# PetarKirov/Chess2RT

Measured on AMD Instinct MI355X. Metric: Mray/s (reference-equivalent rays per second: one primary ray per sample + one shadow ray per (hit, lit light), counted as the reference casts them; ms/frame in ms_per_step), higher is better.
Workload: dtype f64; 1 GPU; lecture5.sdl 3840x2160, 5 tap(s)/pixel (AAEnabled as shipped: reference 5-tap AA), dof off; primary_rays_per_frame=41472000, full=False

## Files before the change

### chess2rt_amd/csrc/c2rt_device.h

```cpp
#ifndef C2RT_DEVICE_H
#define C2RT_DEVICE_H

#include <stddef.h>
#include <stdint.h>

#include "../../include/c2rt.h"
#include "csg_void.h"

namespace c2rt {

constexpr int kMaxCsgHits = C2RT_MAX_CSG_HITS;
constexpr int kCsgEntries = 2 * kMaxCsgHits;
constexpr int kTileW = 8, kTileH = 8;
constexpr int kWave = 64;
inline size_t padded_grid_blocks(uint32_t tile_rows, uint32_t blocks_x) { return (size_t)((tile_rows + 7u) / 8u * 8u) * blocks_x; }
constexpr int kMaxCullNodes = 32;
constexpr int kHullEdges = 6;
constexpr int kMaxCullLights = 4;
constexpr int kWavesPerBlock = 1;
constexpr int kBlockThreads = kWave * kWavesPerBlock;
constexpr int kCsgLdsPerEntry = kWave * (8 + 2);
constexpr int kCsgFullCap(int levels) { return kCsgEntries * (levels > 0 ? levels : 1); }
constexpr int kCsgFirstCap(int levels) { return levels <= 2 ? 16 : 20; }
static_assert(3 * kWavesPerBlock * kCsgFirstCap(C2RT_MAX_CSG_DEPTH) * kCsgLdsPerEntry <= 160 * 1024, "three workgroups per CU");

enum GeomFlags : int32_t {
    kGeomBounded = 1,
    kCsgShortA = 2,
    kCsgShortB = 4,
    kGeomFinite = 8,
    kCsgCertain = 16,
};

struct alignas(16) DevGeom {
    int32_t type, left, right;
    int32_t flags;
    double p[4];
    double bound[4];
    double q[6];
};

enum NodeFlags : uint32_t {
    kNodeIdentityMatrix = 1u,
    kNodeZeroOffset = 2u,
    kNodeAxisPlane = 4u,
    kNodePlaneNormal = 8u,
    kNodeCsgTile = 16u,
};

struct alignas(16) DevMat {
    int32_t shader_type;
    int32_t tex_type;
    int32_t tex;
    float strength;
    float color[3];
    uint32_t pad;
    double exponent;
    uint32_t pad2[2];
    uint32_t texdata[8];
};

struct alignas(16) DevNode {
    int32_t geom, shader;
    uint32_t flags, pad;
    double off[3];
    double pad2;
    DevGeom g;
    double inv[9];
    double m[9];
    double tinv[9];
    double pad3;
    DevMat mat;
};

struct alignas(16) DevShader {
    int32_t type, tex;
    float color[3];
    float strength;
    double exponent;
};

struct alignas(16) DevTex {
    int32_t type;
    uint32_t width, height;
    float scaling;
    uint64_t offset;
    float color[18];
    double param[6];
};

struct alignas(16) DevLight {
    double pos[3];
    float color[3];
    uint32_t lit;
    uint32_t equal;
    uint32_t pad;
};

struct RenderParams {
    const DevGeom *geoms;
    const DevNode *nodes;
    const DevShader *shaders;
    const DevTex *textures;
    const DevLight *lights;
// ... 89 lines not shown
```

### chess2rt_amd/csrc/c2rt_kernels.hip

```cpp
#include "c2rt_trace_common.inc"

namespace c2rt {
namespace {

constexpr int kLeanMaxLevels = 3;

template <int LEVELS, int DOF, bool MLC, int PO, bool CNT>
DEV void render_one(const RenderParams &P, KArgs K, const uint32_t b)
{
    if constexpr (CNT || LEVELS > kLeanMaxLevels) {
        exact::render_tile<LEVELS, DOF, MLC, PO, CNT>(P, K, b);
    } else {
        if (!P.force_exact) {
            const bool redo = lean::render_tile<LEVELS, DOF, MLC, PO, false>(P, K, b);
            if (!__ballot(redo)) return;
            if (threadIdx.x % kWave == 0) atomicAdd(P.redo_counter, 1ull);
        }
        if constexpr (LEVELS <= 1 && !DOF && PO != kSpecPlanes) {
            KArgs K2 = K;
            uint32_t b2 = b;
            asm volatile("" : "+s"(K2), "+s"(b2));
            exact::render_tile<LEVELS, DOF, MLC, PO, false>(*(const RenderParams *)K2, K2, b2);
        } else {
            exact::render_tile<LEVELS, DOF, MLC, PO, false>(P, K, b);
// ... 86 lines not shown

#if C2RT_UNIT == 5
__global__ void deinterleave_kernel(const float *__restrict__ gathered, float *__restrict__ frame,
                                    uint32_t row_floats, uint32_t strip_height, uint32_t world, uint32_t rows_pad)
{
    const uint32_t y = blockIdx.y;
    const uint32_t strip = y / strip_height;
    const uint32_t rank = strip % world;
    const uint32_t lr = (strip / world) * strip_height + y % strip_height;
    const float *src = gathered + ((size_t)rank * rows_pad + lr) * (size_t)row_floats;
    float *dst = frame + (size_t)y * row_floats;
    if ((row_floats & 3u) == 0) {
        const float4 *s4 = reinterpret_cast<const float4 *>(src);
        float4 *d4 = reinterpret_cast<float4 *>(dst);
        for (uint32_t i = blockIdx.x * blockDim.x + threadIdx.x; i < row_floats / 4; i += gridDim.x * blockDim.x) d4[i] = s4[i];
    } else {
        for (uint32_t i = blockIdx.x * blockDim.x + threadIdx.x; i < row_floats; i += gridDim.x * blockDim.x) dst[i] = src[i];
    }
}

__global__ void encode_rgb32_kernel(const float *__restrict__ frame, uint32_t *__restrict__ out, uint64_t n,
                                    const uint8_t *__restrict__ lut)
{
    for (uint64_t i = (uint64_t)blockIdx.x * blockDim.x + threadIdx.x; i < n; i += (uint64_t)gridDim.x * blockDim.x) {
        uint32_t ch[3];
#pragma unroll
        for (int c = 0; c < 3; ++c) {
            const float x = frame[3 * i + c];
            ch[c] = !(x > 0) ? 0u : (x >= 1 ? 255u : (uint32_t)lut[(int)(x * 4096.0f)]);
        }
        out[i] = ch[2] | (ch[1] << 8) | (ch[0] << 16);
    }
}

DEV void tile_masks_body(const RenderParams &P, KArgs K, const VoidCull &V, const SphereCull &S, const DarkCull *D, uint32_t *table, uint32_t tile_rows)
{
    const uint32_t i = blockIdx.x * blockDim.x + threadIdx.x;
    const uint32_t cols = P.blocks_x * kWavesPerBlock;
    const uint32_t trow = i / cols, tcol = i % cols;
    if (trow >= tile_rows) return;
    uint32_t m[8];
    tile_mask_entry(P, K, V, S, D, trow, tcol, m);
    typedef uint32_t __attribute__((ext_vector_type(4))) u4_t;
    u4_t v, w;
    v.x = m[0]; v.y = m[1]; v.z = m[2]; v.w = m[3];
    w.x = m[4]; w.y = m[5]; w.z = m[6]; w.w = m[7];
    const size_t slot = tile_mask_slot(P, trow, tcol);
    reinterpret_cast<u4_t *>(table)[slot] = v;
    if (P.n_cull_lights > 1u) reinterpret_cast<u4_t *>(table)[(size_t)P.mask_entries + slot] = w;
}

static_assert(sizeof(RenderParams) + sizeof(VoidCull) + sizeof(SphereCull) + 24 <= 4096, "the kernel-argument segment holds at most 4 KiB");
__global__ void __launch_bounds__(256) tile_masks_kernel(const RenderParams P, const VoidCull V, const SphereCull S, const DarkCull *dark,
                                                         uint32_t *__restrict__ table, uint32_t tile_rows)
{
    const DarkCull C2RT_K *D = (const DarkCull C2RT_K *)dark;
    tile_masks_body(P, (KArgs)__builtin_amdgcn_kernarg_segment_ptr(), V, S, (const DarkCull *)D, table, tile_rows);
}

__global__ void __launch_bounds__(256) tile_masks_batch_kernel(const RenderParams *table, const BatchCull *culls)
{
    const KArgs K = batch_block(table);
    const BatchCull C2RT_K *C = (const BatchCull C2RT_K *)culls + blockIdx.y;
    asm volatile("" : "+s"(C));
    const RenderParams &P = *(const RenderParams *)K;
    if (!P.n_cull || !P.tile_masks) return;
    const BatchCull &B = *(const BatchCull *)C;
    tile_masks_body(P, K, B.v, B.s, &B.d, const_cast<uint32_t *>(P.tile_masks), (P.mask_rows + kTileH - 1) / kTileH);
}
#endif

}

#ifndef C2RT_UNIT
#error "compile with -DC2RT_UNIT=0..5 (see Makefile)"
#endif

#if C2RT_UNIT >= 0 && C2RT_UNIT <= C2RT_MAX_CSG_DEPTH

static uint32_t frame_grid_x(const RenderParams &p)
{
    return p.retry_mode ? 2048u : (uint32_t)padded_grid_blocks(p.tiles_y, p.blocks_x);
}
static size_t frame_lds(const RenderParams &p) { return (size_t)p.csg_cap * kCsgLdsPerEntry * kWavesPerBlock; }

template <>
int launch_render_level<C2RT_UNIT>(const RenderParams &p, bool dof_or_stereo, void *stream)
{
    hipStream_t s = static_cast<hipStream_t>(stream);
    const dim3 grid(frame_grid_x(p)), block(kBlockThreads);
    const size_t lds = frame_lds(p);
    const bool stereo = p.cam.stereo_separation != 0;
    const bool multi = p.n_lights > 1;
    const bool idn = p.all_identity && !p.ray_counters;
#define C2RT_LAUNCH(KERNEL, ...)                                                                        \
    do {                                                                                                \
        if (p.ray_counters) hipLaunchKernelGGL((KERNEL<__VA_ARGS__, true>), grid, block, lds, s, p);    \
        else hipLaunchKernelGGL((KERNEL<__VA_ARGS__, false>), grid, block, lds, s, p);                  \
    } while (0)
#if C2RT_UNIT == 0
    if (p.planes_only && !multi) {
        if (dof_or_stereo && stereo) C2RT_LAUNCH(render_kernel_planes, 2);
        else if (dof_or_stereo) C2RT_LAUNCH(render_kernel_planes, 1);
        else C2RT_LAUNCH(render_kernel_planes, 0);
        return (int)hipGetLastError();
    }
#endif
    if (dof_or_stereo) {
        if (stereo) C2RT_LAUNCH(render_kernel_dof, C2RT_UNIT, true, 2);
        else if (multi) C2RT_LAUNCH(render_kernel_dof, C2RT_UNIT, true, 1);
        else C2RT_LAUNCH(render_kernel_dof, C2RT_UNIT, false, 1);
    } else if (multi) {
        C2RT_LAUNCH(render_kernel, C2RT_UNIT, 0, true);
    } else if (idn) {
        hipLaunchKernelGGL((render_kernel_idn<C2RT_UNIT>), grid, block, lds, s, p);
    } else {
        C2RT_LAUNCH(render_kernel, C2RT_UNIT, 0, false);
    }
#undef C2RT_LAUNCH
    return (int)hipGetLastError();
}

template <>
int launch_render_batch_level<C2RT_UNIT>(const RenderParams &p0, const RenderParams *table_dev, uint32_t n_frames, void *stream)
{
    hipStream_t s = static_cast<hipStream_t>(stream);
    const dim3 grid(frame_grid_x(p0), n_frames), block(kBlockThreads);
    const size_t lds = frame_lds(p0);
#if C2RT_UNIT == 0
    if (p0.planes_only && p0.n_lights <= 1) {
        hipLaunchKernelGGL(render_kernel_planes_batch, grid, block, lds, s, table_dev);
        return (int)hipGetLastError();
    }
#endif
    if (p0.n_lights > 1) hipLaunchKernelGGL((render_kernel_batch<C2RT_UNIT, true>), grid, block, lds, s, table_dev);
    else if (p0.all_identity) hipLaunchKernelGGL((render_kernel_idn_batch<C2RT_UNIT>), grid, block, lds, s, table_dev);
    else hipLaunchKernelGGL((render_kernel_batch<C2RT_UNIT, false>), grid, block, lds, s, table_dev);
    return (int)hipGetLastError();
}

#elif C2RT_UNIT == 5

int launch_render_batch(const RenderParams &p0, const KernelVariant &v, const RenderParams *table_dev, uint32_t n_frames, void *stream)
{
    if (v.dof_or_stereo || p0.ray_counters || !n_frames || n_frames > 65535u) return (int)hipErrorInvalidValue;
    return for_csg_levels(v.csg_levels, [&](auto L) { return launch_render_batch_level<decltype(L)::value>(p0, table_dev, n_frames, stream); });
}

int launch_tile_masks_batch(const RenderParams &p0, const RenderParams *table_dev, const BatchCull *culls_dev, uint32_t n_frames, void *stream)
{
    const uint32_t tile_rows = (p0.mask_rows + kTileH - 1) / kTileH;
    const uint32_t lanes = tile_rows * p0.blocks_x * kWavesPerBlock;
    if (!lanes || !n_frames) return 0;
    hipLaunchKernelGGL(tile_masks_batch_kernel, dim3((lanes + 255u) / 256u, n_frames), dim3(256), 0, static_cast<hipStream_t>(stream), table_dev, culls_dev);
    return (int)hipGetLastError();
}

int launch_render(const RenderParams &p, const KernelVariant &v, void *stream)
{
    return for_csg_levels(v.csg_levels, [&](auto L) { return launch_render_level<decltype(L)::value>(p, v.dof_or_stereo, stream); });
}

size_t tile_mask_entries(const RenderParams &p)
{
    const uint32_t tile_rows = (p.mask_rows + kTileH - 1) / kTileH;
    return padded_grid_blocks(tile_rows, p.blocks_x) * kWavesPerBlock;
}
// ... 45 lines not shown
```

### chess2rt_amd/csrc/c2rt_trace.inc

```

DEV void len_inv(Oob &bad, double s, double &len, double &inv)
{
    if constexpr (kLean) {
        oob_note_nonneg(bad, s);
        inv_len(s, len, inv);
    } else {
        len = sqrt(s);
        inv = 1.0 / len;
    }
}
DEV void len_inv_unit(Oob &bad, double s, double &len, double &inv)
{
    if constexpr (kLean) {
        if (__all(near_one(s))) {
            unit_len(s, len, inv);
            return;
        }
    }
    len_inv(bad, s, len, inv);
}
DEV double sqrt_g(Oob &bad, double x)
{
    if constexpr (kLean) {
        oob_note(bad, x);
// ... 878 lines not shown
        if (closest >= 0) col_ = shade<LEVELS, MLC, PO>(P, cx, mat, d, surf, cnt.shadow);
#endif
        C2RT_REGION_END(cx, kRegShade)
        return col_;
    }
#endif
    if (closest < 0) return mkf(0, 0, 0);
#if C2RT_CSG_CERTAIN
    return shade<LEVELS, MLC, PO>(P, cx, mat, d, surf, cnt.shadow, closest);
#else
    return shade<LEVELS, MLC, PO>(P, cx, mat, d, surf, cnt.shadow);
#endif
}

template <int LEVELS>
DEV int trace_closest(const Ctx &cx, D3 o, D3 d, bool record, Hit &best, Surf &surf, Mat &mat)
{
    const uint32_t nn = cx.n_nodes;
    best.dist = 1e99;
    best.g = -1;
    best.code = 0;
    best.p = mk(0, 0, 0);
    surf.p = surf.n = mk(0, 0, 0);
    surf.u = surf.v = 0;
    int closest = -1;
    const RayW ray = make_ray(cx.bad, o, d);
    for (uint32_t n = 0; n < nn; ++n)
        if (node_intersect<LEVELS, kFull, 0>(cx, cx.nodes + n, ray, best, n + 1 >= nn && !record)) closest = (int)n;
    mat.tex_type = -1;
    bool todo = closest >= 0;
    while (todo) {
        const int cn = __builtin_amdgcn_readfirstlane(closest);
        if (closest == cn) {
            NodeP N = cx.nodes + cn;
            load_mat(N, mat);
            hit_surface<0>(cx, N, best, uv_want(record || mat.tex_type >= 0), surf);
            todo = false;
        }
    }
    return closest;
}

template <int LEVELS, int DOF, bool MLC, int PO>
DEV F3 render_sample(const RenderParams &P, const Ctx &cx, double x, double y, int dx, int dy, uint64_t pixel, uint32_t tap,
                     Counters &cnt, c2rt_trace_result *probe)
{
    Rng rng = {DOF ? rng_key(P.seed, pixel, tap) : 0u, 0, 0};
    D3 o, d;
    if constexpr (!DOF) {
        screen_ray<false>(cx.bad, P, x, y, 0, rng, o, d);
        return raytrace<LEVELS, MLC, PO>(P, cx, o, d, cnt, probe);
    } else {
        const bool stereo = DOF == 2 && P.cam.stereo_separation != 0;
        const bool dof = P.cam.dof != 0;
        const uint32_t ns = dof ? P.cam.num_samples : 1u;
        const int eyes = stereo ? 2 : 1;
        F3 average = mkf(0, 0, 0), sample = mkf(0, 0, 0);
        for (uint32_t i = 0; i < ns; ++i) {
            rng.sample = i;
            rng.dim = 0;
            KArgs Ks = cx.kargs;
            asm volatile("" : "+s"(Ks));
            const RenderParams &Ps = *(const RenderParams *)Ks;
            for (int e = 0; e < eyes; ++e) {
                double sx = x, sy = y;
                if (dof) {
                    const double jx = rng_next(rng), jy = rng_next(rng);
                    sx = x + jx * dx;
                    sy = y + jy * dy;
                }
                screen_ray<DOF>(cx.bad, Ps, sx, sy, stereo ? (e == 0 ? -1 : +1) : 0, rng, o, d);
                const F3 c = raytrace<LEVELS, MLC, PO>(Ps, cx, o, d, cnt, e == 0 ? probe : nullptr);
                sample = e == 0 ? c : combine_stereo(sample, c);
            }
            if (!dof) return sample;
            average = average + sample;
        }
        return average / (float)ns;
    }
}

__constant__ double k_aa_x[5] = {0.0, 0.3, 0.6, 0.0, 0.6};
__constant__ double k_aa_y[5] = {0.0, 0.3, 0.0, 0.6, 0.6};

template <int PO>
DEV int ground_tile(const RenderParams &P, KArgs K, const uint32_t trow, const uint32_t bcol, const bool dark)
{
    static_assert(!(PO & kSpecPlanes), "the planes-only instances have no mask table");
    const int lane = threadIdx.x & (kWave - 1);
    const int wave = threadIdx.x / kWave;
    const uint32_t tcol = bcol * kWavesPerBlock + wave;
    const uint32_t x = tcol * kTileW + (lane % kTileW);
    const uint32_t lr0 = trow * kTileH + (lane / kTileW);
    if (x >= P.width || lr0 >= P.local_rows) return kGroundDone;
    const uint32_t lr = lr0 + P.row_offset;
    const uint32_t y = frame_row(P, lr);
    const uint32_t ntaps = P.taps;

    Oob bad;
    oob_init(bad);
    F3 accum = mkf(0, 0, 0);
#pragma unroll 1
    for (uint32_t s = 0; s < ntaps; ++s) {
        KArgs Kt = K;
        asm volatile("" : "+s"(Kt));
        const RenderParams &Pt = *(const RenderParams *)Kt;
        Rng rng = {0u, 0, 0};
        D3 o, raw;
        screen_ray<0>(bad, Pt, (double)x + k_aa_x[s], (double)y + k_aa_y[s], 0, rng, o, raw);
        const D3 d = normalized(bad, raw);
        NodeP N = (NodeP)Pt.nodes + Pt.ground_node;
        double len, inv;
        len_inv_unit(bad, sqmag(d), len, inv);
        const D3 dn = mk(d.x * inv, d.y * inv, d.z * inv);
        const double gy = N->g.p[0], limit = N->g.p[1];
        const bool away = ((o.y > gy) & (dn.y > -1e-9)) | ((o.y < gy) & (dn.y < 1e-9));
        const double rden = rcp_refined(-dn.y);
        const double mult = div_r(bad, o.y - gy, -dn.y, rden);
        const D3 p = o + dn * mult;
        const bool miss = away | (mult > 1e99 * len) | (fabs(p.x) > limit) | (fabs(p.z) > limit);
        F3 c = mkf(0, 0, 0);
        bool bail = false;
        if (!miss) {
            Mat mat;
            load_mat(N, mat);
            const F3 diffuse = mat.tex_type == C2RT_TEX_CHECKER ? checker_color(mat, p.x, p.z)
                             : (mat.tex_type >= 0 ? bitmap_color(Pt, mat, p.x, p.z) : mat.color);
            F3 lightContrib = mkf(Pt.ambient[0], Pt.ambient[1], Pt.ambient[2]);
            if (dark) {
                lightContrib = lightContrib + mkf(0, 0, 0);
            } else if (Pt.n_lights) {
                LightP L = (LightP)Pt.lights;
                F3 avgColor = mkf(0, 0, 0);
                if (L->lit & 1u) {
                    const bool up = d.y < 0;
                    const D3 lightPos = ld3(L->pos);
                    const double from_y = p.y + (up ? 1e-6 : -1e-6);
                    const D3 lv = lightPos - p;
                    const double r2 = sqmag(lv);
                    double rlen, rinv;
                    len_inv(bad, r2, rlen, rinv);
                    const double ldy = lv.y * rinv;
                    const double cosTheta = up ? ldy : -ldy;
                    const F3 baseLight = base_light(bad, L, r2);
                    const double raw_y = lightPos.y - from_y, ground_y = Pt.ground_y;
                    const bool sane = (fabs(lv.x) < 1e150) & (fabs(lv.z) < 1e150);
                    const bool rises = (raw_y > 1e-150) & (raw_y < 1e150), falls = (raw_y < -1e-150) & (raw_y > -1e150);
                    bail = !__all(sane & (((from_y > ground_y) & rises) | ((from_y < ground_y) & falls)));
                    if (cosTheta > 0) avgColor = avgColor + baseLight * (float)cosTheta;
                }
                lightContrib = lightContrib + avgColor;
            }
            c = diffuse * lightContrib;
        }
        if (__ballot(bail)) return kGroundBail;
        accum = s == 0 ? c : accum + c;
    }
    if (ntaps > 1) accum = accum / (float)ntaps;
    if (__ballot(oob_any(bad))) return kGroundRedo;
    store_pixel(P, (size_t)(P.frame_rows ? y : lr) * P.width + x, accum);
    return kGroundDone;
}

template <int PO>
DEV int ground_tile_certain(const RenderParams &P, KArgs K, const uint32_t trow, const uint32_t bcol, const bool dark)
{
    static_assert(!(PO & kSpecPlanes), "the planes-only instances have no mask table");
    const int lane = threadIdx.x & (kWave - 1);
    const int wave = threadIdx.x / kWave;
    const uint32_t tcol = bcol * kWavesPerBlock + wave;
    const uint32_t x = tcol * kTileW + (lane % kTileW);
    const uint32_t lr0 = trow * kTileH + (lane / kTileW);
    if (x >= P.width || lr0 >= P.local_rows) return kGroundDone;
    const uint32_t lr = lr0 + P.row_offset;
    const uint32_t y = frame_row(P, lr);
    const uint32_t ntaps = P.taps;

    Oob bad;
    oob_init(bad);
    bool unsure = false;
    F3 accum = mkf(0, 0, 0);
#pragma unroll 1
    for (uint32_t s = 0; s < ntaps; ++s) {
        KArgs Kt = K;
        asm volatile("" : "+s"(Kt));
        const RenderParams &Pt = *(const RenderParams *)Kt;
        Rng rng = {0u, 0, 0};
        D3 o, raw;
        screen_ray<0>(bad, Pt, (double)x + k_aa_x[s], (double)y + k_aa_y[s], 0, rng, o, raw);
        NodeP N = (NodeP)Pt.nodes + Pt.ground_node;
        const double gy = N->g.p[0], limit = N->g.p[1];
        double px, pz, bx, bz, q;
        const int state = gc_hit(o.x, o.z, o.y - gy, raw.x, raw.y, raw.z, (double)Pt.ground_certain_cq, limit, &px, &pz, &bx, &bz, &q);
        bool u = state == GC_UNSURE;
        F3 c = mkf(0, 0, 0);
        if (state == GC_HIT) {
            Mat mat;
            load_mat(N, mat);
            F3 diffuse = mat.color;
            if (mat.tex_type >= 0) {
                const double sc = (double)__uint_as_float(mat.td[2]);
                float fu, fv;
                u |= !gc_tex_float(px, bx, sc, &fu);
                u |= !gc_tex_float(pz, bz, sc, &fv);
                const uint32_t w = mat.td[0], hgt = mat.td[1];
                diffuse = bitmap_filtered_uniform(Pt.texels, mat.td[4], w, hgt, fu * (float)w, fv * (float)hgt);
            }
            F3 lightContrib = mkf(Pt.ambient[0], Pt.ambient[1], Pt.ambient[2]);
            if (dark) {
                lightContrib = lightContrib + mkf(0, 0, 0);
            } else if (Pt.n_lights) {
                LightP L = (LightP)Pt.lights;
                F3 avgColor = mkf(0, 0, 0);
                if (L->lit & 1u) {
                    const gc_frame f = gc_frame_of(0.0, 1, L->pos[1], gy);
                    float r2f, cosf;
                    double unread[4];
                    u |= !gc_light(px, pz, q, L->pos[0], L->pos[2], &f, &r2f, &cosf, unread);
                    if (L->equal) {
                        oob_note_f32(bad, r2f);
                        const float b = div_with_f32(L->color[0], r2f, rcp_refined_f32(r2f));
                        const float a = 0.0f + b * cosf;
                        avgColor = mkf(a, a, a);
                    } else {
                        avgColor = avgColor + base_light(bad, L, (double)r2f) * cosf;
                    }
                }
                lightContrib = lightContrib + avgColor;
            }
            c = diffuse * lightContrib;
        }
        unsure |= u;
        accum = s == 0 ? c : accum + c;
    }
    if (ntaps > 1) tap_average(bad, accum, (float)ntaps);
    if (__ballot(unsure | oob_any(bad))) {
        if (lane == (int)__builtin_ctzll(__ballot(true))) atomicAdd(P.redo_counter + 1, 1ull);
        return kGroundBail;
    }
    store_pixel(P, (size_t)(P.frame_rows ? y : lr) * P.width + x, accum);
    return kGroundDone;
}

template <int PO>
DEV int sphere_tile(const RenderParams &P, KArgs K, const uint32_t trow, const uint32_t bcol, const uint32_t node)
{
    static_assert(!(PO & kSpecPlanes), "the planes-only instances have no mask table");
    const int lane = threadIdx.x & (kWave - 1);
    const int wave = threadIdx.x / kWave;
    const uint32_t tcol = bcol * kWavesPerBlock + wave;
    const uint32_t x = tcol * kTileW + (lane % kTileW);
    const uint32_t lr0 = trow * kTileH + (lane / kTileW);
    if (x >= P.width || lr0 >= P.local_rows) return kGroundDone;
    const uint32_t lr = lr0 + P.row_offset;
    const uint32_t y = frame_row(P, lr);
    const uint32_t ntaps = P.taps;

    Oob bad;
    oob_init(bad);
    bool missed = false;
    F3 accum = mkf(0, 0, 0);
#pragma unroll 1
    for (uint32_t s = 0; s < ntaps; ++s) {
        KArgs Kt = K;
        asm volatile("" : "+s"(Kt));
        const RenderParams &Pt = *(const RenderParams *)Kt;
        Rng rng = {0u, 0, 0};
        D3 o, raw;
        screen_ray<0>(bad, Pt, (double)x + k_aa_x[s], (double)y + k_aa_y[s], 0, rng, o, raw);
        const D3 d = normalized(bad, raw);
        NodeP N = (NodeP)Pt.nodes + node;
        GeomP G = &N->g;
        const bool has_off = !(N->flags & kNodeZeroOffset);
        const RayW ray = make_ray(bad, o, d);
        Hit h;
        {
            ORay rc;
            rc.o = ray.o;
            if (has_off) rc.o = rc.o - ld3(N->off);
            rc.d = ray.dn;
            rc.A = ray.A;
            prep_dir(rc, kPrepA);
            h.dist = 1e99 * ray.len;
            h.p = ray.o;
            missed |= !sphere_intersect<kFull>(bad, G, N->geom, rc, h, false);
        }
        Mat mat;
        load_mat(N, mat);
        const D3 pc = h.p - ld3(G->p);
        D3 n = normalized(bad, pc);
        F3 diffuse = mat.color;
        if (mat.tex_type >= 0) {
            double u, v;
            const double sc = (double)__uint_as_float(mat.td[2]);
            sphere_uv(pc.x, pc.z, pc.y / G->p[3], UVWant{kUVBitmap, sc}, u, v);
            u *= sc;
            v *= sc;
            u = u - floor(u);
            v = v - floor(v);
            const uint32_t w = mat.td[0], hgt = mat.td[1];
            diffuse = bitmap_filtered_uniform(Pt.texels, mat.td[4], w, hgt, (float)u * (float)w, (float)v * (float)hgt);
// ... 194 lines not shown
                                if (test_c && visible) visible = !node_intersect<1, kBool, PO>(cx, Nc, sray, temp, false, on_c);
                            }
                        }
                        if (visible) {
                            if (cosTheta > 0) avgColor = avgColor + baseLight * (float)cosTheta;
                            if (phong & (cosGamma > 0))
                                avgSpecular = avgSpecular + baseLight * c2_pow_f32(cosGamma, Mc->exponent) * Mc->strength;
                        }
                    }
                }
                lightContrib = lightContrib + avgColor;
                specular = specular + avgSpecular;
            }
            const F3 res = diffuse * lightContrib;
            c = phong ? res + specular : res;
        }
        accum = s == 0 ? c : accum + c;
    }
    if (ntaps > 1) accum = accum / (float)ntaps;
    if (__ballot(cx.overflow)) {
        if (lane == (int)__builtin_ctzll(__ballot(true))) atomicAdd(P.redo_counter + 3, 1ull);
        return kGroundBail;
    }
    if (__ballot(oob_any(cx.bad))) return kGroundRedo;
    store_pixel(P, (size_t)(P.frame_rows ? y : lr) * P.width + x, accum);
#if C2RT_TILE_STATS
    if (lane == (int)__builtin_ctzll(__ballot(true))) {
        atomicAdd(P.redo_counter + 4, 1ull);
        if (P.tile_stats) {
            const unsigned long long dt = __builtin_amdgcn_s_memtime() - stamp0;
            const uint32_t tile = trow * P.tiles_x + tcol;
            P.tile_stats[2 * tile] = dt > 0xFFFFFFFFull ? 0xFFFFFFFFu : (uint32_t)dt;
            P.tile_stats[2 * tile + 1] = ((1u << P.ground_node) | (1u << node)) << 8;
        }
    }
#endif
    return kGroundDone;
}
#endif

template <int LEVELS, int DOF, bool MLC, int PO, bool CNT>
DEV bool render_tile(const RenderParams &P, KArgs K, const uint32_t b)
{
    extern __shared__ __align__(16) char lds_all[];
    const int lane = threadIdx.x & (kWave - 1);
    const int wave = threadIdx.x / kWave;
    char *lds = lds_all + (size_t)wave * P.csg_cap * kCsgLdsPerEntry;

    const uint32_t xcd = b & 7u, j = b >> 3;
    const uint32_t groups = (P.tiles_y + 7u) / 8u;
    uint32_t grp = j / P.blocks_x + P.row_group_start;
    if (grp >= groups) grp -= groups;
    const uint32_t trow = grp * 8u + xcd, bcol = j % P.blocks_x;
    if (trow >= P.tiles_y) return false;
    const uint32_t tcol = bcol * kWavesPerBlock + wave;
#if C2RT_TILE_STATS
    const unsigned long long stamp0 = __builtin_amdgcn_s_memtime();
#endif

    uint32_t pmask = 0xFFFFFFFFu, smask0 = 0xFFFFFFFFu, mask_slot = 0;
    bool ground_only = false, primary_ground = false, dark = false, interior = false;
    Oob tile_bad;
    oob_init(tile_bad);
    if constexpr (!DOF) {
        if (P.n_cull) {
            typedef uint32_t __attribute__((ext_vector_type(4))) u4_t;
            mask_slot = (uint32_t)tile_mask_slot(P, trow + (P.row_offset - P.mask_row0) / kTileH, (uint32_t)__builtin_amdgcn_readfirstlane(tcol));
            const u4_t m = ((const u4_t C2RT_K *)P.tile_masks)[mask_slot];
            pmask = m.x;
            smask0 = m.y;
            primary_ground = (m.z & 1u) != 0;
            ground_only = (m.z & 2u) != 0;
            dark = (m.z & 4u) != 0;
            interior = (m.z & 8u) != 0;
        }
    }

    if constexpr (kLean && LEVELS <= 1 && !DOF && !MLC && !CNT && !(PO & kSpecPlanes) && !C2RT_TILE_STATS) {
        if (P.ground_fast && (ground_only || dark)) {
            KArgs Kg = K;
            uint32_t trow_g = trow, bcol_g = bcol, dark_g = (uint32_t)__builtin_amdgcn_readfirstlane(dark && !ground_only ? 1 : 0);
            asm volatile("" : "+s"(Kg), "+s"(trow_g), "+s"(bcol_g), "+s"(dark_g));
            if (((const RenderParams *)Kg)->ground_certain_cq > 0) {
                const int gc = ground_tile_certain<PO>(*(const RenderParams *)Kg, Kg, trow_g, bcol_g, dark_g != 0);
                if (!__ballot(gc == kGroundBail)) return false;
                asm volatile("" : "+s"(Kg), "+s"(trow_g), "+s"(bcol_g), "+s"(dark_g));
            }
            const int g = ground_tile<PO>(*(const RenderParams *)Kg, Kg, trow_g, bcol_g, dark_g != 0);
            if (!__ballot(g == kGroundBail)) return g == kGroundRedo;
        }
        if (__builtin_expect(interior, 0)) {
            uint32_t rest = pmask & (0xFFFFFFFFu >> (32u - P.n_nodes));
            if (P.ground_node >= 0) rest &= ~(1u << P.ground_node);
            KArgs Ks = K;
            uint32_t trow_s = trow, bcol_s = bcol, node_s = (uint32_t)__builtin_amdgcn_readfirstlane((int)__builtin_ctz(rest | 0x80000000u));
            asm volatile("" : "+s"(Ks), "+s"(trow_s), "+s"(bcol_s), "+s"(node_s));
            const int g = sphere_tile<PO>(*(const RenderParams *)Ks, Ks, trow_s, bcol_s, node_s);
            if (!__ballot(g == kGroundBail)) return g == kGroundRedo;
        }
    }
#if C2RT_CSG_TILE
    if constexpr (kLean && LEVELS == 1 && !DOF && !MLC && !CNT && (PO & kSpecIdentity) && !(PO & kSpecPlanes)) {
        if (P.ground_fast && !ground_only && P.n_nodes <= 32u) {
            const uint32_t live = 0xFFFFFFFFu >> (32u - P.n_nodes), gbit = 1u << P.ground_node;
            const uint32_t pm = pmask & live, sm = smask0 & live, rest = pm & ~gbit;
            if (__builtin_expect((pm & gbit) && rest && !(rest & (rest - 1u)) && !(sm & ~pm), 0)) {
                uint32_t node_c = (uint32_t)__builtin_amdgcn_readfirstlane((int)__builtin_ctz(rest));
                if (((NodeP)P.nodes)[node_c].flags & kNodeCsgTile) {
                    KArgs Kc = K;
                    uint32_t trow_c = trow, bcol_c = bcol, smask_c = (uint32_t)__builtin_amdgcn_readfirstlane((int)sm);
                    asm volatile("" : "+s"(Kc), "+s"(trow_c), "+s"(bcol_c), "+s"(node_c), "+s"(smask_c));
                    const int g = csg_tile<PO>(*(const RenderParams *)Kc, Kc, trow_c, bcol_c, node_c, smask_c);
                    if (!__ballot(g == kGroundBail)) return g == kGroundRedo;
                }
            }
        }
    }
#endif

    if (P.n_nodes == 1u && P.ground_node == 0) primary_ground = true;

    const uint32_t x = tcol * kTileW + (lane % kTileW);
    const uint32_t lr0 = trow * kTileH + (lane / kTileW);
    if (x >= P.width || lr0 >= P.local_rows) return false;
    const uint32_t lr = lr0 + P.row_offset;

    uint32_t y = lr;
    if (P.strip_world > 1) {
        const uint32_t sh = P.strip_height;
        y = ((lr / sh) * P.strip_world + P.strip_rank) * sh + lr % sh;
    }

    Ctx cx;
    cx.geoms = (GeomP)P.geoms;
    cx.nodes = (NodeP)P.nodes;
    cx.n_nodes = P.n_nodes;
    cx.kargs = K;
    cx.lds = lds;
    cx.lane = lane;
    cx.csg_cap = (int)P.csg_cap;
    cx.overflow = false;
    cx.bad = tile_bad;
    cx.trunc_counter = CNT ? P.ray_counters + 2 : nullptr;
#if C2RT_CSG_CERTAIN
    cx.csg_certain = !CNT;
#endif
#if C2RT_TILE_STATS
    cx.lane_stats = P.tile_stats ? reinterpret_cast<unsigned long long *>(P.tile_stats + 2 * (size_t)P.tiles_x * P.tiles_y) : nullptr;
#endif
    cx.block = b;
    cx.mask_slot = mask_slot;
    cx.primary_mask = pmask;
    cx.shadow_mask0 = smask0;
    cx.shadow_ground_only = ground_only;
    cx.primary_ground_only = primary_ground;
    cx.ground_y = P.ground_y;
    Counters cnt = {0, 0};
    uint32_t sx = x, sy = y;
    int jdx = 1, jdy = 1;
    if (P.prepass_bucket) {
        const uint32_t bs = P.prepass_bucket;
        const uint32_t bx = x / bs * bs, by = y / bs * bs;
        sx = bx + ((x - bx) & ~15u);
        sy = by + ((y - by) & ~15u);
        const uint32_t bx1 = bx + bs < P.width ? bx + bs : P.width, by1 = by + bs < P.height ? by + bs : P.height;
        jdx = (int)(sx + 16u < bx1 ? 16u : bx1 - sx);
        jdy = (int)(sy + 16u < by1 ? 16u : by1 - sy);
// ... 67 lines not shown
```

### chess2rt_amd/csrc/c2rt_trace_shared.inc

```
#define C2RT_K __attribute__((address_space(4)))
typedef const DevGeom C2RT_K *GeomP;
typedef const DevNode C2RT_K *NodeP;
typedef const DevLight C2RT_K *LightP;
typedef const DevTex C2RT_K *TexP;
typedef const DevMat C2RT_K *MatP;
typedef const double C2RT_K *KDbl;
typedef const float C2RT_K *KFlt;

#if C2RT_TILE_STATS
enum { kRegTrace = 0, kRegCsg = 1, kRegReplay = 2, kRegSurface = 3, kRegShade = 4, kRegShadow = 5, kRegTexture = 6, kRegLight = 7, kRegSphereUV = 8, kRegions = 9 };
#define C2RT_REGION_BEGIN(cx, id)                                                                          \
    const unsigned long long rs_##id = (cx).lane_stats ? __builtin_amdgcn_s_memtime() : 0ull;              \
    const unsigned long long ra_##id = __ballot(true);
#define C2RT_REGION_END(cx, id)                                                                            \
    if ((cx).lane_stats) {                                                                                 \
        const unsigned long long now_ = __builtin_amdgcn_s_memtime();                                      \
        if ((cx).lane == (int)__builtin_ctzll(__ballot(true))) {                                           \
            atomicAdd((cx).lane_stats + 4 + 3 * (id) + 0, now_ - rs_##id);                                 \
            atomicAdd((cx).lane_stats + 4 + 3 * (id) + 1, (unsigned long long)__builtin_popcountll(ra_##id)); \
            atomicAdd((cx).lane_stats + 4 + 3 * (id) + 2, 64ull);                                          \
        }                                                                                                  \
    }
#else
#define C2RT_REGION_BEGIN(cx, id)
// ... 134 lines not shown
#endif
#if C2RT_TILE_STATS
    cx.lane_stats = nullptr;
#endif
    cx.block = 0;
    cx.mask_slot = 0;
    cx.primary_mask = 0xFFFFFFFFu;
    cx.shadow_mask0 = 0xFFFFFFFFu;
    cx.shadow_ground_only = false;
    cx.primary_ground_only = false;
    cx.ground_y = 0;
}

DEV int next_gap(int inc)
{
    static_assert(2 * kMaxCsgHits <= 22, "gap * 5 / 11 in integers");
    return inc == 2 ? 1 : (inc * 5) / 11;
}

static_assert(kMaxCsgHits <= 8 && C2RT_MAX_CSG_GEOMS <= 4096, "16-bit hit tags");
DEV uint16_t csg_tag(int leaf, int side, int k) { return (uint16_t)(((uint32_t)leaf << 4) | ((uint32_t)side << 3) | (uint32_t)k); }

DEV uint32_t next_node(uint32_t mask, uint32_t n)
{
    static_assert(kMaxCullNodes == 32, "one 32-bit mask");
    if (n >= 32u) return n;
    const uint32_t m = mask >> n;
    return m ? n + (uint32_t)__builtin_ctz(m) : 32u;
}

DEV bool plane_points_away(NodeP N, D3 from, D3 raw)
{
    const uint32_t fl = N->flags;
    double oy = (fl & kNodeZeroOffset) ? from.y : from.y - N->off[1];
    if (!(fl & kNodeIdentityMatrix)) {
        const double ox = (fl & kNodeZeroOffset) ? from.x : from.x - N->off[0];
        const double oz = (fl & kNodeZeroOffset) ? from.z : from.z - N->off[2];
        oy = ox * N->inv[1] + oy * N->inv[4] + oz * N->inv[7];
    }
    const double y = N->g.p[0];
    const bool sane = (fabs(raw.x) < 1e150) & (fabs(raw.z) < 1e150);
    const bool up = (raw.y > 1e-150) & (raw.y < 1e150), down = (raw.y < -1e-150) & (raw.y > -1e150);
    return sane & (((oy > y) & up) | ((oy < y) & down));
}

enum { kSpecPlanes = 1, kSpecIdentity = 2 };

enum { kUVNone = 0, kUVExact = 1, kUVBitmap = 2 };
struct UVWant {
    int kind;
    double s;
};
DEV UVWant uv_want(bool exact) { return UVWant{exact ? kUVExact : kUVNone, 0.0}; }

DEV void sphere_uv(double dx, double dz, double w, UVWant want, double &u, double &v)
{
    const UV r = want.kind == kUVBitmap ? c2_sphere_uv_bitmap(dx, dz, w, want.s) : c2_sphere_uv(dx, dz, w);
    u = r.u;
    v = r.v;
}


DEV F3 bitmap_filtered(const float4 *texels, uint32_t width, uint32_t height, float x, float y)
{
    if (!(x < (float)width) | !(y < (float)height) | (width == 0) | (height == 0))
        return mkf(1.0f, 0.0f, 0.0f);
    const float fx = floorf(x), fy = floorf(y);
    const uint32_t tx = (uint32_t)fx, ty = (uint32_t)fy;
    const uint32_t txn = tx + 1 == width ? 0 : tx + 1;
    const uint32_t tyn = ty + 1 == height ? 0 : ty + 1;
    const float p = x - fx, q = y - fy;
    const float4 c00 = texels[(size_t)ty * width + tx], c10 = texels[(size_t)ty * width + txn];
    const float4 c01 = texels[(size_t)tyn * width + tx], c11 = texels[(size_t)tyn * width + txn];
    const float w00 = (1.0f - p) * (1.0f - q), w10 = p * (1.0f - q), w01 = (1.0f - p) * q, w11 = p * q;
    return mkf(c00.x, c00.y, c00.z) * w00 + mkf(c10.x, c10.y, c10.z) * w10 + mkf(c01.x, c01.y, c01.z) * w01 +
           mkf(c11.x, c11.y, c11.z) * w11;
}

DEV float alone(float v)
{
    asm("" : "+v"(v));
    return v;
}
DEV F3 bitmap_filtered_uniform(const float *pool, uint32_t offset, uint32_t width, uint32_t height, float x, float y)
{
    if (!(x < (float)width) | !(y < (float)height) | (width == 0) | (height == 0))
        return mkf(1.0f, 0.0f, 0.0f);
    typedef float __attribute__((ext_vector_type(2))) f2_t;
    typedef float __attribute__((ext_vector_type(3))) f3_t;
    const float fx = floorf(x), fy = floorf(y);
    const uint32_t tx = (uint32_t)fx, ty = (uint32_t)fy;
    const uint32_t txn = tx + 1 == width ? 0 : tx + 1;
    const float p = x - fx, q = y - fy;
    const uint32_t row0 = __umul24(ty, width) + offset;
    const uint32_t row1 = ty + 1 == height ? offset : row0 + width;
    const char __attribute__((address_space(1))) *base = (const char __attribute__((address_space(1))) *)pool;
#define C2RT_TEXEL(i) (*(const f3_t __attribute__((address_space(1))) *)(base + (uint64_t)(uint32_t)((i) << 4)))
    const f3_t c00 = C2RT_TEXEL(row0 + tx), c10 = C2RT_TEXEL(row0 + txn);
    const f3_t c01 = C2RT_TEXEL(row1 + tx), c11 = C2RT_TEXEL(row1 + txn);
#undef C2RT_TEXEL
    const float w00 = alone((1.0f - p) * (1.0f - q)), w10 = alone(p * (1.0f - q)), w01 = alone((1.0f - p) * q), w11 = alone(p * q);
    const float b = ((alone(c00.z * w00) + alone(c10.z * w10)) + alone(c01.z * w01)) + alone(c11.z * w11);
    const f2_t rg = ((c00.xy * w00 + c10.xy * w10) + c01.xy * w01) + c11.xy * w11;
    return mkf(rg.x, rg.y, b);
}

struct Mat {
    int shader_type, tex_type, tex;
    float strength;
    F3 color;
    double exponent;
    uint32_t td[8];
};

DEV void load_mat(NodeP N, Mat &m)
{
    MatP M = &N->mat;
    m.shader_type = M->shader_type;
    m.tex_type = M->tex_type;
    m.tex = M->tex;
    m.strength = M->strength;
    m.color = ldf3(M->color);
    m.exponent = M->exponent;
#pragma unroll
    for (int i = 0; i < 8; ++i) m.td[i] = M->texdata[i];
}

DEV F3 checker_color(const Mat &m, double u, double v)
{
    const double size = __hiloint2double((int)m.td[7], (int)m.td[6]);
    const int x = d2i_x86(floor(u / size));
    const int y = d2i_x86(floor(v / size));
    const int white = (int)((uint32_t)x + (uint32_t)y) % 2;
    return white ? mkf(__uint_as_float(m.td[3]), __uint_as_float(m.td[4]), __uint_as_float(m.td[5]))
                 : mkf(__uint_as_float(m.td[0]), __uint_as_float(m.td[1]), __uint_as_float(m.td[2]));
}

DEV F3 bitmap_color(const RenderParams &P, const Mat &m, double u, double v)
{
    const double s = (double)__uint_as_float(m.td[2]);
    u *= s;
    v *= s;
    u = u - floor(u);
    v = v - floor(v);
    const uint32_t w = m.td[0], hgt = m.td[1];
    const float tx = (float)u * (float)w;
    const float ty = (float)v * (float)hgt;
    const uint64_t offset = (uint64_t)m.td[4] | ((uint64_t)m.td[5] << 32);
    return bitmap_filtered(reinterpret_cast<const float4 *>(P.texels) + offset, w, hgt, tx, ty);
}

DEV F3 tex_color(const RenderParams &P, const Mat &m, double u, double v)
{
    const int type = m.tex_type;
    if (type == C2RT_TEX_CHECKER) {
        return checker_color(m, u, v);
    } else if (type == C2RT_TEX_PROCEDURE2) {
        TexP T = (TexP)P.textures + m.tex;
        F3 result = mkf(0, 0, 0);
#pragma unroll
        for (int i = 0; i < 3; ++i)
            result = result + (ldf3(T->color + 3 * i) * (float)c2_sin(u * T->param[i]) +
                               ldf3(T->color + 9 + 3 * i) * (float)c2_sin(v * T->param[3 + i]));
        return result;
    } else {
        return bitmap_color(P, m, u, v);
    }
}

DEV uint32_t hash32(uint32_t x)
{
    x ^= x >> 16;
    x *= 0x7feb352du;
    x ^= x >> 15;
    x *= 0x846ca68bu;
    x ^= x >> 16;
    return x;
}
DEV uint32_t rng_key(uint64_t seed, uint64_t pixel, uint32_t tap)
{
    uint32_t k = hash32((uint32_t)(seed >> 32) ^ 0x243f6a88u);
    k = hash32(k ^ (uint32_t)seed);
    k = hash32(k + (uint32_t)(pixel >> 32));
    k = hash32(k ^ (uint32_t)pixel);
    return hash32(k + tap);
}
DEV double rng_uniform(uint32_t key, uint32_t sample, uint32_t dim)
// ... 98 lines not shown
```

### chess2rt_amd/csrc/ground_certain.h

```cpp
#ifndef C2RT_GROUND_CERTAIN_H
#define C2RT_GROUND_CERTAIN_H

#include <math.h>

#if defined(__HIPCC__)
#define GC_FN static __host__ __device__ __forceinline__
#else
#define GC_FN static inline
#endif

#if defined(__HIP_DEVICE_COMPILE__)
#define GC_FMA(a, b, c) __builtin_fma((a), (b), (c))
#define GC_RCP_SEED(b) __builtin_amdgcn_rcp(b)
#define GC_RSQ_SEED(x) __builtin_amdgcn_rsq(x)
#else
#define GC_FMA(a, b, c) fma((a), (b), (c))
#ifndef GC_SEED_SCALE
#define GC_SEED_SCALE (1.0 + 0x1p-24)
#endif
#define GC_RCP_SEED(b) ((1.0 / (b)) * (GC_SEED_SCALE))
#define GC_RSQ_SEED(x) ((1.0 / sqrt(x)) * (GC_SEED_SCALE))
#endif

#define GC_U 0x1p-53
#define GC_KP 12.0
#define GC_KQ2 58.0
#define GC_KR2 6.1
#define GC_KH 16.0
#define GC_KCY 138.0
#define GC_KCU 79.0

enum { GC_HIT = 0, GC_MISS = 1, GC_UNSURE = 2 };

typedef struct {
    double cq;
    double h, h2;
} gc_frame;

GC_FN double gc_rcp(double b)
{
    const double r0 = GC_RCP_SEED(b);
    const double e = GC_FMA(-b, r0, 1.0);
    const double p = GC_FMA(e, e, e);
    return GC_FMA(r0, p, r0);
}

GC_FN double gc_rsq(double x)
{
    const double y0 = GC_RSQ_SEED(x);
    const double t = x * y0;
    const double e = GC_FMA(-t, y0, 1.0);
    const double p = GC_FMA(e, 0.375, 0.5);
    const double pe = p * e;
    return GC_FMA(y0, pe, y0);
}

GC_FN float gc_plan(const double o[3], double gy, double limit, int lit, const double L[3], int textured, double s)
{
    const double A = o[1] - gy;
    if (!((A >= 0x1p-40) & (A <= 0x1p20) & (fabs(o[0]) <= 0x1p40) & (fabs(o[2]) <= 0x1p40) & (fabs(gy) <= 0x1p20) & !(limit <= 0))) return 0;
    if (textured && !((fabs(s) >= 0x1p-40) & (fabs(s) <= 0x1p40))) return 0;
    double cq = 2 * fabs(o[0]) + 2 * fabs(o[2]) + 0x1p-100;
    if (lit) {
        const double h = L[1] - gy;
        if (!((h >= 0x1p-17) & (h <= 0x1p20) & (fabs(L[0]) <= 0x1p40) & (fabs(L[2]) <= 0x1p40) & (A <= GC_KH * h) & (fabs(gy) <= GC_KH * h))) return 0;
        cq += fabs(L[0]) + fabs(L[2]);
    }
    return (float)(cq * (1 + 0x1p-20));
}

GC_FN gc_frame gc_frame_of(double cq, int lit, double ly, double gy)
{
    gc_frame f;
    f.cq = cq;
    f.h = lit ? ly - gy : 0.0;
    f.h2 = f.h * f.h;
    return f;
}

GC_FN int gc_hit(double ox, double oz, double A, double rx, double ry, double rz, double cq, double limit,
                 double *px, double *pz, double *bx, double *bz, double *q)
{
    const double m1 = fabs(rx) + fabs(ry) + fabs(rz);
    const int win = (m1 >= 0x1p-90) & (m1 < 0x1p90);
    const int away = ry >= 0;
    const int hit = -ry > 1.001e-9 * m1;
    const double t = A * gc_rcp(-ry);
    *px = GC_FMA(rx, t, ox);
    *pz = GC_FMA(rz, t, oz);
    const double ax = fabs(*px), az = fabs(*pz);
    *bx = GC_FMA(ax, GC_KP * GC_U, GC_FMA(fabs(ox), 2 * GC_KP * GC_U, fmin(fabs(rx) * 0x1p150, 0x1p-650)));
    *bz = GC_FMA(az, GC_KP * GC_U, GC_FMA(fabs(oz), 2 * GC_KP * GC_U, fmin(fabs(rz) * 0x1p150, 0x1p-650)));
    *q = ax + az + cq;
    const int in = !((ax + *bx >= limit) | (az + *bz >= limit));
    const int out = (ax - *bx > limit) | (az - *bz > limit);
    if (!win) return GC_UNSURE;
    if (away) return GC_MISS;
    if (!hit) return GC_UNSURE;
    return in ? GC_HIT : (out ? GC_MISS : GC_UNSURE);
}

GC_FN int gc_tex_float(double pp, double b, double s, float *out)
{
    const double a0 = (pp - b) * s, a1 = (pp + b) * s;
    const double f0 = floor(a0), f1 = floor(a1);
    const float x0 = (float)(a0 - f0), x1 = (float)(a1 - f1);
    *out = x0;
    return (f0 == f1) & (x0 == x1);
}

GC_FN int gc_light(double px, double pz, double q, double lx, double lz, const gc_frame *f, float *r2f, float *cosf, double dbg[4])
{
    const double lvx = lx - px, lvz = lz - pz;
    const double r2 = GC_FMA(lvx, lvx, GC_FMA(lvz, lvz, f->h2));
    const double E = GC_FMA(q * q, GC_KQ2 * GC_U, f->h2 * (GC_KCY * GC_U));
    const double B = GC_FMA(r2, GC_KR2 * GC_U, E);
    const float lo = (float)(r2 - B), hi = (float)(r2 + B);
    const double y1 = gc_rsq(r2);
    const double c = f->h * y1;
    const double rel = GC_FMA(E * (y1 * y1), 0.504, GC_KCU * GC_U);
    const double bc = c * rel;
    const float clo = (float)(c - bc), chi = (float)(c + bc);
    dbg[0] = r2;
    dbg[1] = B;
    dbg[2] = c;
    dbg[3] = bc;
    *r2f = lo;
    *cosf = clo;
    return (lo == hi) & (rel < 0x1p-22) & (clo == chi);
}

#endif
```

Baseline: 172,300 Mray/s.

## Share per-column/row AA ray terms via LDS in certain-ground tile path

In the certain-ground fast path for multi-tap AA, each 8x8 tile now precomputes the camera x-terms (per column and AA offset) and y-terms (per row and AA offset) once into LDS. Each tap's ray direction is then assembled from two LDS reads instead of a full screen_ray computation with divides. Loop-invariant ground and light quantities (height, cq, texture scale and size, light frame) are hoisted out of the tap loop, and an unlimited-plane variant of gc_hit skips the bounds test. This adds LDS use and a wavefront fence for the one-wave workgroups. It also relies on the fixed 5-tap offset pattern.

```diff
diff --git a/chess2rt_amd/csrc/c2rt_device.h b/chess2rt_amd/csrc/c2rt_device.h
--- a/chess2rt_amd/csrc/c2rt_device.h
+++ b/chess2rt_amd/csrc/c2rt_device.h
@@ -20,6 +20,7 @@
 constexpr int kWavesPerBlock = 1;
 constexpr int kBlockThreads = kWave * kWavesPerBlock;
 constexpr int kCsgLdsPerEntry = kWave * (8 + 2);
+constexpr int kRayTermsLds = 2 * kTileW * 3 * 3 * 8;
 constexpr int kCsgFullCap(int levels) { return kCsgEntries * (levels > 0 ? levels : 1); }
 constexpr int kCsgFirstCap(int levels) { return levels <= 2 ? 16 : 20; }
 static_assert(3 * kWavesPerBlock * kCsgFirstCap(C2RT_MAX_CSG_DEPTH) * kCsgLdsPerEntry <= 160 * 1024, "three workgroups per CU");
diff --git a/chess2rt_amd/csrc/c2rt_kernels.hip b/chess2rt_amd/csrc/c2rt_kernels.hip
--- a/chess2rt_amd/csrc/c2rt_kernels.hip
+++ b/chess2rt_amd/csrc/c2rt_kernels.hip
@@ -192,7 +192,11 @@
 {
     return p.retry_mode ? 2048u : (uint32_t)padded_grid_blocks(p.tiles_y, p.blocks_x);
 }
-static size_t frame_lds(const RenderParams &p) { return (size_t)p.csg_cap * kCsgLdsPerEntry * kWavesPerBlock; }
+static size_t frame_lds(const RenderParams &p)
+{
+    const size_t stack = (size_t)p.csg_cap * kCsgLdsPerEntry, terms = C2RT_UNIT <= 1 ? (size_t)kRayTermsLds : 0;
+    return (stack > terms ? stack : terms) * kWavesPerBlock;
+}
 
 template <>
 int launch_render_level<C2RT_UNIT>(const RenderParams &p, bool dof_or_stereo, void *stream)
diff --git a/chess2rt_amd/csrc/c2rt_trace.inc b/chess2rt_amd/csrc/c2rt_trace.inc
--- a/chess2rt_amd/csrc/c2rt_trace.inc
+++ b/chess2rt_amd/csrc/c2rt_trace.inc
@@ -984,6 +984,60 @@
 
 __constant__ double k_aa_x[5] = {0.0, 0.3, 0.6, 0.0, 0.6};
 __constant__ double k_aa_y[5] = {0.0, 0.3, 0.0, 0.6, 0.6};
+
+constexpr double kAaOffset[3] = {0.0, 0.3, 0.6};
+constexpr uint32_t kAaIx = 0x20210u, kAaIy = 0x22010u;
+constexpr bool aa_offsets_match()
+{
+    constexpr double ax[5] = {0.0, 0.3, 0.6, 0.0, 0.6}, ay[5] = {0.0, 0.3, 0.0, 0.6, 0.6};
+    for (int s = 0; s < 5; ++s)
+        if (kAaOffset[(kAaIx >> (4 * s)) & 3u] != ax[s] || kAaOffset[(kAaIy >> (4 * s)) & 3u] != ay[s]) return false;
+    return true;
+}
+static_assert(aa_offsets_match(), "kAaIx / kAaIy index the AA kernel's offsets");
+static_assert(kWavesPerBlock == 1 && kTileW == 8 && kTileH == 8, "ray terms: one wave per workgroup, lanes 0..23 and 32..55 of an 8x8 tile");
+
+typedef double __attribute__((address_space(3))) *LdsDbl;
+
+struct RayTerms {
+    uint32_t ax, by;
+};
+
+DEV RayTerms ray_terms_setup(const RenderParams &P, LdsDbl t, const int lane, const uint32_t trow, const uint32_t tcol)
+{
+    const c2rt_camera_frame &cam = P.cam;
+    const uint32_t k = (uint32_t)lane & 7u, i = ((uint32_t)lane >> 3) & 3u;
+    const double off = i == 0 ? kAaOffset[0] : (i == 1 ? kAaOffset[1] : kAaOffset[2]);
+    const uint32_t entry = (k * 3u + i) * 3u;
+    if (lane < 24) {
+        const uint32_t x = tcol * kTileW + k;
+        const double fx = div_with((double)x + off, cam.frame_width, P.cam_rw);
+        const D3 a = ld3(cam.up_left) + ld3(P.cam_du) * fx;
+        t[entry] = a.x;
+        t[entry + 1] = a.y;
+        t[entry + 2] = a.z;
+    } else if (lane >= 32 && lane < 56) {
+        const uint32_t y = frame_row(P, trow * kTileH + k + P.row_offset);
+        const double fy = div_with((double)y + off, cam.frame_height, P.cam_rh);
+        const D3 b = ld3(P.cam_dv) * fy;
+        t[kRayTermsLds / 16 + entry] = b.x;
+        t[kRayTermsLds / 16 + entry + 1] = b.y;
+        t[kRayTermsLds / 16 + entry + 2] = b.z;
+    }
+    __builtin_amdgcn_fence(__ATOMIC_ACQ_REL, "wavefront");
+    RayTerms r;
+    r.ax = ((uint32_t)lane & 7u) * 9u;
+    r.by = kRayTermsLds / 16 + ((uint32_t)lane >> 3) * 9u;
+    return r;
+}
+
+DEV D3 ray_terms_dir(LdsDbl t, const RayTerms r, const uint32_t s, const D3 pos)
+{
+    const uint32_t ia = r.ax + ((kAaIx >> (4u * s)) & 3u) * 3u, ib = r.by + ((kAaIy >> (4u * s)) & 3u) * 3u;
+    const D3 a = mk(t[ia], t[ia + 1], t[ia + 2]), b = mk(t[ib], t[ib + 1], t[ib + 2]);
+    const D3 target = a + b;
+    return target - pos;
+}
 
 template <int PO>
 DEV int ground_tile(const RenderParams &P, KArgs K, const uint32_t trow, const uint32_t bcol, const bool dark)
@@ -1064,19 +1118,44 @@
     return kGroundDone;
 }
 
-template <int PO>
+template <int PO, bool SHARED>
 DEV int ground_tile_certain(const RenderParams &P, KArgs K, const uint32_t trow, const uint32_t bcol, const bool dark)
 {
     static_assert(!(PO & kSpecPlanes), "the planes-only instances have no mask table");
+    extern __shared__ __align__(16) char lds_all[];
+    const LdsDbl terms = (LdsDbl)lds_all;
     const int lane = threadIdx.x & (kWave - 1);
     const int wave = threadIdx.x / kWave;
     const uint32_t tcol = bcol * kWavesPerBlock + wave;
+    RayTerms rt = {0u, 0u};
+    if constexpr (SHARED) rt = ray_terms_setup(P, terms, lane, trow, tcol);
     const uint32_t x = tcol * kTileW + (lane % kTileW);
     const uint32_t lr0 = trow * kTileH + (lane / kTileW);
     if (x >= P.width || lr0 >= P.local_rows) return kGroundDone;
     const uint32_t lr = lr0 + P.row_offset;
     const uint32_t y = frame_row(P, lr);
     const uint32_t ntaps = P.taps;
+
+    double A = 0, cq = 0, sc = 0, cy = 0;
+    float wf = 0, hf = 0;
+    gc_frame f = gc_frame_of(0.0, 0, 0.0, 0.0);
+    if constexpr (SHARED) {
+        NodeP N0 = (NodeP)P.nodes + P.ground_node;
+        const double gy0 = N0->g.p[0];
+        A = P.cam.pos[1] - gy0;
+        cq = (double)P.ground_certain_cq;
+        if (N0->mat.tex_type >= 0) {
+            sc = (double)__uint_as_float(N0->mat.texdata[2]);
+            wf = (float)N0->mat.texdata[0];
+            hf = (float)N0->mat.texdata[1];
+        }
+        if (!dark && P.n_lights) {
+            LightP L0 = (LightP)P.lights;
+            if (L0->lit & 1u) f = gc_frame_of(0.0, 1, L0->pos[1], gy0);
+        }
+        cy = f.h2 * (GC_KCY * GC_U);
+        asm volatile("" : "+v"(A), "+v"(cq), "+v"(sc), "+v"(wf), "+v"(hf), "+v"(f.h), "+v"(f.h2), "+v"(cy));
+    }
 
     Oob bad;
     oob_init(bad);
@@ -1087,13 +1166,30 @@
         KArgs Kt = K;
         asm volatile("" : "+s"(Kt));
         const RenderParams &Pt = *(const RenderParams *)Kt;
-        Rng rng = {0u, 0, 0};
         D3 o, raw;
-        screen_ray<0>(bad, Pt, (double)x + k_aa_x[s], (double)y + k_aa_y[s], 0, rng, o, raw);
+        if constexpr (SHARED) {
+            o = ld3(Pt.cam.pos);
+            raw = ray_terms_dir(terms, rt, s, o);
+        } else {
+            Rng rng = {0u, 0, 0};
+            screen_ray<0>(bad, Pt, (double)x + k_aa_x[s], (double)y + k_aa_y[s], 0, rng, o, raw);
+        }
         NodeP N = (NodeP)Pt.nodes + Pt.ground_node;
-        const double gy = N->g.p[0], limit = N->g.p[1];
+        if constexpr (!SHARED) {
+            A = o.y - N->g.p[0];
+            cq = (double)Pt.ground_certain_cq;
+        }
+        const uint64_t limit_bits = (uint64_t)__double_as_longlong(N->g.p[1]);
+        const bool unlimited = (limit_bits & 0x7FFFFFFFFFFFFFFFull) > 0x7FF0000000000000ull;
         double px, pz, bx, bz, q;
-        const int state = gc_hit(o.x, o.z, o.y - gy, raw.x, raw.y, raw.z, (double)Pt.ground_certain_cq, limit, &px, &pz, &bx, &bz, &q);
+        int state;
+        if (unlimited) {
+            state = gc_hit_unlimited(o.x, o.z, A, raw.x, raw.y, raw.z, cq, &px, &pz, &bx, &bz, &q);
+        } else {
+            double limit = N->g.p[1];
+            asm volatile("" : "+v"(limit));
+            state = gc_hit(o.x, o.z, A, raw.x, raw.y, raw.z, cq, limit, &px, &pz, &bx, &bz, &q);
+        }
         bool u = state == GC_UNSURE;
         F3 c = mkf(0, 0, 0);
         if (state == GC_HIT) {
@@ -1101,12 +1197,16 @@
             load_mat(N, mat);
             F3 diffuse = mat.color;
             if (mat.tex_type >= 0) {
-                const double sc = (double)__uint_as_float(mat.td[2]);
+                if constexpr (!SHARED) {
+                    sc = (double)__uint_as_float(mat.td[2]);
+                    wf = (float)mat.td[0];
+                    hf = (float)mat.td[1];
+                }
                 float fu, fv;
                 u |= !gc_tex_float(px, bx, sc, &fu);
                 u |= !gc_tex_float(pz, bz, sc, &fv);
                 const uint32_t w = mat.td[0], hgt = mat.td[1];
-                diffuse = bitmap_filtered_uniform(Pt.texels, mat.td[4], w, hgt, fu * (float)w, fv * (float)hgt);
+                diffuse = bitmap_filtered_uniform(Pt.texels, mat.td[4], w, hgt, wf, hf, fu * wf, fv * hf);
             }
             F3 lightContrib = mkf(Pt.ambient[0], Pt.ambient[1], Pt.ambient[2]);
             if (dark) {
@@ -1115,10 +1215,13 @@
                 LightP L = (LightP)Pt.lights;
                 F3 avgColor = mkf(0, 0, 0);
                 if (L->lit & 1u) {
-                    const gc_frame f = gc_frame_of(0.0, 1, L->pos[1], gy);
+                    if constexpr (!SHARED) {
+                        f = gc_frame_of(0.0, 1, L->pos[1], N->g.p[0]);
+                        cy = f.h2 * (GC_KCY * GC_U);
+                    }
                     float r2f, cosf;
                     double unread[4];
-                    u |= !gc_light(px, pz, q, L->pos[0], L->pos[2], &f, &r2f, &cosf, unread);
+                    u |= !gc_light_cy(px, pz, q, L->pos[0], L->pos[2], &f, cy, &r2f, &cosf, unread);
                     if (L->equal) {
                         oob_note_f32(bad, r2f);
                         const float b = div_with_f32(L->color[0], r2f, rcp_refined_f32(r2f));
@@ -1479,7 +1582,9 @@
             uint32_t trow_g = trow, bcol_g = bcol, dark_g = (uint32_t)__builtin_amdgcn_readfirstlane(dark && !ground_only ? 1 : 0);
             asm volatile("" : "+s"(Kg), "+s"(trow_g), "+s"(bcol_g), "+s"(dark_g));
             if (((const RenderParams *)Kg)->ground_certain_cq > 0) {
-                const int gc = ground_tile_certain<PO>(*(const RenderParams *)Kg, Kg, trow_g, bcol_g, dark_g != 0);
+                const int gc = ((const RenderParams *)Kg)->taps > 1u
+                                   ? ground_tile_certain<PO, true>(*(const RenderParams *)Kg, Kg, trow_g, bcol_g, dark_g != 0)
+                                   : ground_tile_certain<PO, false>(*(const RenderParams *)Kg, Kg, trow_g, bcol_g, dark_g != 0);
                 if (!__ballot(gc == kGroundBail)) return false;
                 asm volatile("" : "+s"(Kg), "+s"(trow_g), "+s"(bcol_g), "+s"(dark_g));
             }
diff --git a/chess2rt_amd/csrc/c2rt_trace_shared.inc b/chess2rt_amd/csrc/c2rt_trace_shared.inc
--- a/chess2rt_amd/csrc/c2rt_trace_shared.inc
+++ b/chess2rt_amd/csrc/c2rt_trace_shared.inc
@@ -240,9 +240,9 @@
     asm("" : "+v"(v));
     return v;
 }
-DEV F3 bitmap_filtered_uniform(const float *pool, uint32_t offset, uint32_t width, uint32_t height, float x, float y)
-{
-    if (!(x < (float)width) | !(y < (float)height) | (width == 0) | (height == 0))
+DEV F3 bitmap_filtered_uniform(const float *pool, uint32_t offset, uint32_t width, uint32_t height, float wf, float hf, float x, float y)
+{
+    if (!(x < wf) | !(y < hf) | (width == 0) | (height == 0))
         return mkf(1.0f, 0.0f, 0.0f);
     typedef float __attribute__((ext_vector_type(2))) f2_t;
     typedef float __attribute__((ext_vector_type(3))) f3_t;
@@ -261,6 +261,11 @@
     const float b = ((alone(c00.z * w00) + alone(c10.z * w10)) + alone(c01.z * w01)) + alone(c11.z * w11);
     const f2_t rg = ((c00.xy * w00 + c10.xy * w10) + c01.xy * w01) + c11.xy * w11;
     return mkf(rg.x, rg.y, b);
+}
+
+DEV F3 bitmap_filtered_uniform(const float *pool, uint32_t offset, uint32_t width, uint32_t height, float x, float y)
+{
+    return bitmap_filtered_uniform(pool, offset, width, height, (float)width, (float)height, x, y);
 }
 
 struct Mat {
diff --git a/chess2rt_amd/csrc/ground_certain.h b/chess2rt_amd/csrc/ground_certain.h
--- a/chess2rt_amd/csrc/ground_certain.h
+++ b/chess2rt_amd/csrc/ground_certain.h
@@ -78,8 +78,8 @@
     return f;
 }
 
-GC_FN int gc_hit(double ox, double oz, double A, double rx, double ry, double rz, double cq, double limit,
-                 double *px, double *pz, double *bx, double *bz, double *q)
+GC_FN int gc_hit_unlimited(double ox, double oz, double A, double rx, double ry, double rz, double cq,
+                           double *px, double *pz, double *bx, double *bz, double *q)
 {
     const double m1 = fabs(rx) + fabs(ry) + fabs(rz);
     const int win = (m1 >= 0x1p-90) & (m1 < 0x1p90);
@@ -92,11 +92,19 @@
     *bx = GC_FMA(ax, GC_KP * GC_U, GC_FMA(fabs(ox), 2 * GC_KP * GC_U, fmin(fabs(rx) * 0x1p150, 0x1p-650)));
     *bz = GC_FMA(az, GC_KP * GC_U, GC_FMA(fabs(oz), 2 * GC_KP * GC_U, fmin(fabs(rz) * 0x1p150, 0x1p-650)));
     *q = ax + az + cq;
+    if (!win) return GC_UNSURE;
+    if (away) return GC_MISS;
+    return hit ? GC_HIT : GC_UNSURE;
+}
+
+GC_FN int gc_hit(double ox, double oz, double A, double rx, double ry, double rz, double cq, double limit,
+                 double *px, double *pz, double *bx, double *bz, double *q)
+{
+    const int state = gc_hit_unlimited(ox, oz, A, rx, ry, rz, cq, px, pz, bx, bz, q);
+    const double ax = fabs(*px), az = fabs(*pz);
     const int in = !((ax + *bx >= limit) | (az + *bz >= limit));
     const int out = (ax - *bx > limit) | (az - *bz > limit);
-    if (!win) return GC_UNSURE;
-    if (away) return GC_MISS;
-    if (!hit) return GC_UNSURE;
+    if (state != GC_HIT) return state;
     return in ? GC_HIT : (out ? GC_MISS : GC_UNSURE);
 }
 
@@ -109,11 +117,11 @@
     return (f0 == f1) & (x0 == x1);
 }
 
-GC_FN int gc_light(double px, double pz, double q, double lx, double lz, const gc_frame *f, float *r2f, float *cosf, double dbg[4])
+GC_FN int gc_light_cy(double px, double pz, double q, double lx, double lz, const gc_frame *f, double cy, float *r2f, float *cosf, double dbg[4])
 {
     const double lvx = lx - px, lvz = lz - pz;
     const double r2 = GC_FMA(lvx, lvx, GC_FMA(lvz, lvz, f->h2));
-    const double E = GC_FMA(q * q, GC_KQ2 * GC_U, f->h2 * (GC_KCY * GC_U));
+    const double E = GC_FMA(q * q, GC_KQ2 * GC_U, cy);
     const double B = GC_FMA(r2, GC_KR2 * GC_U, E);
     const float lo = (float)(r2 - B), hi = (float)(r2 + B);
     const double y1 = gc_rsq(r2);
@@ -130,4 +138,9 @@
     return (lo == hi) & (rel < 0x1p-22) & (clo == chi);
 }
 
+GC_FN int gc_light(double px, double pz, double q, double lx, double lz, const gc_frame *f, float *r2f, float *cosf, double dbg[4])
+{
+    return gc_light_cy(px, pz, q, lx, lz, f, f->h2 * (GC_KCY * GC_U), r2f, cosf, dbg);
+}
+
 #endif
```

After: 174,000 Mray/s (median of 6 runs). About the same (+1.0%).
